# BaeHann/feature_level_style_transfer_for_TSC

Measured on AMD Instinct MI355X. Metric: train-step samples/sec (univariate TS, len=512, batch=256) at 1/2/4/8 MI355X, higher is better.
Workload: dtype bf16x3

## Files before the change

feature_level_style_transfer_for_tsc_amd/_lib.py:

```python
from __future__ import annotations

import ctypes
import os
from ctypes import POINTER, Structure, c_char_p, c_float, c_int, c_int32, c_int64, c_void_p
from typing import Optional

import torch

ABI_VERSION = 14
_LIB_NAME = "libfst_hip.so"
_HERE = os.path.dirname(os.path.abspath(__file__))
LIB_PATH = os.environ.get("FST_HIP_LIB", os.path.join(_HERE, _LIB_NAME))


class FstLibraryError(RuntimeError):
    pass


class WSrc(Structure):
    _fields_ = [("w", c_void_p), ("off0", c_int64), ("sm", c_int64), ("sc", c_int64), ("st", c_int64)]


_P = c_void_p
_I32P = c_void_p
_SIGNATURES = {
    "fst_version": (c_int, []),
    "fst_last_error": (c_char_p, []),
    "fst_pack_weights": (c_int, [_I32P, _I32P, c_int, POINTER(WSrc), POINTER(WSrc), c_int, c_int, c_int, c_int, _P, c_void_p]),
    "fst_pack_weights_bf16x3": (c_int, [_I32P, _I32P, c_int, POINTER(WSrc), POINTER(WSrc), c_int, c_int, c_int, c_int, _P, c_void_p]),
    "fst_unpack_weights": (c_int, [_I32P, _I32P, c_int, _P, c_int, _P, c_int64, c_int64, c_int64, c_int64,
                                   _P, c_int64, c_int64, c_int64, c_int64, c_int, c_void_p]),
    "fst_mask_taps": (c_int, [_P, _I32P, _I32P, c_int, c_int, c_int, c_void_p]),
    "fst_conv_gemm": (c_int, [_P, c_int64, _P, c_int64, _P, _I32P, _I32P, c_int, _P, _P, c_int64, _P, c_int64,
                              _P, c_int64, c_int, c_int, c_int, c_int, c_int, c_int, c_int, c_int, c_void_p]),
    "fst_conv_wgrad": (c_int, [_P, c_int64, _P, c_int64, _P, c_int64, _P, c_int64, c_int, _P, _I32P, _I32P, c_int,
                               c_int, c_int, c_int, c_int, c_int, c_int64, c_void_p]),
    "fst_conv_last_route": (c_int, [POINTER(c_int32)]),
    "fst_row_sum": (c_int, [_P, c_int64, c_int, c_int, c_int, _P, c_void_p]),
    "fst_bn_stats": (c_int, [_P, c_int, c_int, c_int, _P, c_int64, c_void_p]),
    "fst_bn_finalize": (c_int, [_P, c_int, _P, _P, _P, _P, c_int, c_int, c_float, c_float, _P, c_void_p]),
    "fst_bn_apply": (c_int, [_P, _P, _P, _P, _P, c_int, c_int, c_int, c_int, c_int64, c_void_p]),
    "fst_bn_bwd_reduce": (c_int, [_P, _P, _P, _P, c_int, c_int, c_int, c_int, _P, c_int64, c_void_p]),
    "fst_bn_bwd_apply": (c_int, [_P, _P, _P, _P, _P, c_int, _P, _P, _P, c_int, c_int, c_int, c_int, c_int, c_int, c_int64, c_void_p]),
    "fst_gate_fwd": (c_int, [_P, _P, c_int, c_int, c_int, c_int64, c_void_p]),
    "fst_gate_bwd": (c_int, [_P, _P, _P, c_int, c_int, c_int, c_int64, c_void_p]),
    "fst_coupling_sum_slots": (c_int64, [c_int, c_int, c_int]),
    "fst_coupling_fwd": (c_int, [_P, _P, _P, c_int, c_int, c_int, c_int64, _P, c_void_p]),
    "fst_coupling_bwd": (c_int, [_P, _P, _P, _P, _P, _P, _P, _P, c_int, c_int, c_int, c_int64, c_void_p]),
    "fst_coupling_inv_fwd": (c_int, [_P, _P, _P, c_int, c_int, c_int, c_int64, c_void_p]),
    "fst_coupling_inv_bwd": (c_int, [_P, _P, _P, _P, _P, c_int, c_int, c_int, c_int64, c_void_p]),
    "fst_rmsprop_multi": (c_int, [_P, _P, _P, _P, _P, c_int, c_float, c_float, c_void_p]),
    "fst_adam_multi": (c_int, [_P, _P, _P, _P, _P, c_int, _P, c_float, c_float, c_float, c_float, c_void_p]),
    "fst_wn_stack_fwd_ok": (c_int, [c_int, c_int, c_int, c_int]),
    "fst_wn_stack_fwd": (c_int, [_P, _P, _P, c_int64, _P, _P, _P, c_int64, _P, c_int, c_int, c_int, c_int, c_int, c_int64, c_void_p]),
    "fst_wn_stack_bwd_ok": (c_int, [c_int, c_int, c_int, c_int]),
    "fst_wn_stack_bwd": (c_int, [_P, _P, _P, _P, _P, _P, _P, _P, _P, c_int64, c_int, c_int, c_int, c_int, c_int, c_int64, c_void_p]),
    "fst_wn_wgrad_ok": (c_int, [c_int, c_int, c_int, c_int, c_int, c_int]),
    "fst_wn_wgrad_workspace_floats": (c_int64, [c_int, c_int, c_int, c_int, c_int, c_int]),
    "fst_wn_wgrad_in": (c_int, [_P, _P, _P, c_int, c_int64, _P, _P, _P, c_int64, c_int, c_int, c_int, c_int, c_int, c_int, c_int64,
                                c_void_p]),
    "fst_wn_wgrad_rs": (c_int, [_P, _P, _P, c_int, _P, _P, c_int64, c_int, c_int, c_int, c_int, c_int64, c_void_p]),
    "fst_nt_gemm_workspace_floats": (c_int64, [c_int, c_int, c_int]),
    "fst_nt_gemm": (c_int, [_P, _P, _P, _P, c_int64, c_int, c_int, c_int, _P, _P, c_int, c_float, _P, c_void_p]),
    "fst_tap_wgrad_ok": (c_int, [c_int, c_int, c_int, c_int, c_int, c_int, c_int]),
    "fst_tap_wgrad_workspace_floats": (c_int64, [c_int, c_int, c_int, c_int, c_int]),
    "fst_tap_wgrad": (c_int, [_P, _P, _P, _P, c_int64, c_int, c_int, c_int, c_int, c_int, c_int, c_int, c_int, c_int64, c_int64, c_void_p]),
# ... 93 lines not shown
```

feature_level_style_transfer_for_tsc_amd/csrc/pointwise.hip:

```cpp
#include "fst_common.h"

static thread_local char g_err[512] = "";
void fst_set_error(const char* fmt, ...) {
  va_list ap;
  va_start(ap, fmt);
  vsnprintf(g_err, sizeof(g_err), fmt, ap);
  va_end(ap);
}
extern "C" const char* fst_last_error(void) { return g_err; }

int fst_allow_full_lds(const void* fn, const char* who) {
  static const void* done[64];
  static int n_done = 0;
  for (int i = 0; i < n_done; ++i)
    if (done[i] == fn) return 0;
  hipError_t e = hipFuncSetAttribute(fn, hipFuncAttributeMaxDynamicSharedMemorySize, 160 * 1024);
  if (e != hipSuccess) {
    fst_set_error("%s: hipFuncSetAttribute: %s", who, hipGetErrorString(e));
    return (int)e;
  }
  if (n_done < 64) done[n_done++] = fn;
  return 0;
}
int fst_cu_count(void) {
// ... 184 lines not shown
    rvar[c] = (1.f - momentum) * rvar[c] + momentum * unbiased;
  } else {
    mean = rmean[c];
    var = rvar[c];
  }
  const float invstd = 1.0f / sqrtf(var + eps);
  const float scale = gamma[c] * invstd;
  stats[c] = mean;
  stats[C + c] = invstd;
  stats[2 * C + c] = scale;
  stats[3 * C + c] = beta[c] - mean * scale;
}

extern "C" int fst_bn_finalize(const float* part, int n_slots, const float* gamma, const float* beta, float* running_mean,
                               float* running_var, int train, int C, float eps, float momentum, float* stats, void* stream) {
  FST_REQUIRE(gamma && beta && running_mean && running_var && stats && C > 0, "fst_bn_finalize: bad arguments");
  FST_REQUIRE(!train || (part && n_slots > 0), "fst_bn_finalize: train mode needs the moment partials (n_slots=%d)", n_slots);
  hipLaunchKernelGGL(bn_finalize_kernel, dim3((C + 63) / 64), dim3(64), 0, (hipStream_t)stream, part, n_slots, gamma, beta,
                     running_mean, running_var, train, C, eps, momentum, stats);
  FST_LAUNCH_CHECK();
  return 0;
}

__global__ __launch_bounds__(256) void bn_apply_kernel(const float* y, const float* stats, const float* res,
                                                       const float* res_stats, float* out, int C, int L, int relu) {
  const int bc = blockIdx.x;
  const int c = bc % C;
  const float sc = stats[2 * C + c], sh = stats[3 * C + c];
  float rsc = 1.f, rsh = 0.f;
  if (res && res_stats) { rsc = res_stats[2 * C + c]; rsh = res_stats[3 * C + c]; }
  const long long base = (long long)bc * L;
  for (int t = threadIdx.x; t < L; t += 256) {
    float v = y[base + t] * sc + sh;
    if (res) v += res[base + t] * rsc + rsh;
    if (relu) v = fmaxf(v, 0.f);
    out[base + t] = v;
  }
}

__global__ __launch_bounds__(256) void bn_apply_vec_kernel(const float* y, const float* stats, const float* res,
                                                           const float* res_stats, float* out, int rows, int C, int L,
                                                           int relu, RowVec rv) {
  const int r = threadIdx.x >> rv.shift, t0 = threadIdx.x & ((1 << rv.shift) - 1), rpp = 256 >> rv.shift;
  const int bc = blockIdx.x * rpp + r;
  if (bc >= rows) return;
  const int c = bc % C;
  const float sc = stats[2 * C + c], sh = stats[3 * C + c];
  float rsc = 1.f, rsh = 0.f;
  if (res && res_stats) { rsc = res_stats[2 * C + c]; rsh = res_stats[3 * C + c]; }
  const long long base = (long long)bc * rv.L4;
  const float4* y4 = reinterpret_cast<const float4*>(y) + base;
  const float4* r4 = res ? reinterpret_cast<const float4*>(res) + base : nullptr;
  float4* o4 = reinterpret_cast<float4*>(out) + base;
  for (int t = t0; t < rv.L4; t += 1 << rv.shift) {
    float4 v = y4[t];
    v.x = v.x * sc + sh; v.y = v.y * sc + sh; v.z = v.z * sc + sh; v.w = v.w * sc + sh;
    if (r4) {
      const float4 q = r4[t];
      v.x += q.x * rsc + rsh; v.y += q.y * rsc + rsh; v.z += q.z * rsc + rsh; v.w += q.w * rsc + rsh;
    }
    if (relu) { v.x = fmaxf(v.x, 0.f); v.y = fmaxf(v.y, 0.f); v.z = fmaxf(v.z, 0.f); v.w = fmaxf(v.w, 0.f); }
    o4[t] = v;
  }
}

extern "C" int fst_bn_apply(const float* y, const float* stats, const float* res, const float* res_stats, float* out,
                            int B, int C, int L, int relu, int64_t numel, void* stream) {
  FST_REQUIRE(y && stats && out && B > 0 && C > 0 && L > 0, "fst_bn_apply: bad arguments");
  FST_REQUIRE_EXTENT("fst_bn_apply", B, C, L, numel);
  if (vec_ok(L, {y, res, out})) {
    const RowVec rv = row_vec(L);
    const int rpp = 256 >> rv.shift;
    hipLaunchKernelGGL(bn_apply_vec_kernel, dim3((B * C + rpp - 1) / rpp), dim3(256), 0, (hipStream_t)stream, y, stats, res,
                       res_stats, out, B * C, C, L, relu, rv);
  } else {
    hipLaunchKernelGGL(bn_apply_kernel, dim3(B * C), dim3(256), 0, (hipStream_t)stream, y, stats, res, res_stats, out, C, L, relu);
  }
  FST_LAUNCH_CHECK();
  return 0;
}

__global__ __launch_bounds__(256) void bn_bwd_reduce_kernel(const float* dy, const float* y, const float* out,
                                                            const float* stats, int B, int C, int L, int relu, float* red) {
  const int c = blockIdx.x;
  const float mean = stats[c], invstd = stats[C + c];
  float s1 = 0.f, s2 = 0.f;
  for (int b = blockIdx.y; b < B; b += gridDim.y) {
    const long long base = ((long long)b * C + c) * L;
    for (int t = threadIdx.x; t < L; t += 256) {
      float g = dy[base + t];
      if (relu && !(out[base + t] > 0.f)) g = 0.f;
      s1 += g;
      s2 += g * (y[base + t] - mean) * invstd;
    }
  }
  block_sum2(s1, s2);
  if (threadIdx.x == 0) {
    red[(long long)c * FST_BN_SLOTS + blockIdx.y] = s1;
    red[((long long)C + c) * FST_BN_SLOTS + blockIdx.y] = s2;
  }
}

__global__ __launch_bounds__(256) void bn_bwd_reduce_vec_kernel(const float* dy, const float* y, const float* out,
                                                                const float* stats, int B, int C, int L, int relu,
                                                                float* red, RowVec rv) {
  const int c = blockIdx.x, r = threadIdx.x >> rv.shift, t0 = threadIdx.x & ((1 << rv.shift) - 1), rpp = 256 >> rv.shift;
  const float mean = stats[c], invstd = stats[C + c];
  float s1 = 0.f, s2 = 0.f;
  for (int b = blockIdx.y + r * gridDim.y; b < B; b += rpp * gridDim.y) {
    const long long base = ((long long)b * C + c) * rv.L4;
    const float4* dy4 = reinterpret_cast<const float4*>(dy) + base;
    const float4* y4 = reinterpret_cast<const float4*>(y) + base;
    const float4* o4 = reinterpret_cast<const float4*>(out) + base;
    for (int t = t0; t < rv.L4; t += 1 << rv.shift) {
      float4 g = dy4[t];
      const float4 v = y4[t];
      if (relu) {
        const float4 o = o4[t];
        if (!(o.x > 0.f)) g.x = 0.f;
        if (!(o.y > 0.f)) g.y = 0.f;
        if (!(o.z > 0.f)) g.z = 0.f;
        if (!(o.w > 0.f)) g.w = 0.f;
      }
      s1 += (g.x + g.y) + (g.z + g.w);
      s2 += (g.x * (v.x - mean) + g.y * (v.y - mean) + g.z * (v.z - mean) + g.w * (v.w - mean)) * invstd;
    }
  }
  block_sum2(s1, s2);
  if (threadIdx.x == 0) {
    red[(long long)c * FST_BN_SLOTS + blockIdx.y] = s1;
    red[((long long)C + c) * FST_BN_SLOTS + blockIdx.y] = s2;
  }
}

extern "C" int fst_bn_bwd_reduce(const float* dy, const float* y, const float* out, const float* stats, int B, int C,
                                 int L, int relu, float* red, int64_t numel, void* stream) {
  FST_REQUIRE(dy && y && stats && red && (!relu || out) && B > 0 && C > 0 && L > 0, "fst_bn_bwd_reduce: bad arguments");
  FST_REQUIRE_EXTENT("fst_bn_bwd_reduce", B, C, L, numel);
  if (vec_ok(L, {dy, y, out}))
    hipLaunchKernelGGL(bn_bwd_reduce_vec_kernel, dim3(C, FST_BN_SLOTS), dim3(256), 0, (hipStream_t)stream, dy,
                       y, out, stats, B, C, L, relu, red, row_vec(L));
  else
    hipLaunchKernelGGL(bn_bwd_reduce_kernel, dim3(C, FST_BN_SLOTS), dim3(256), 0, (hipStream_t)stream, dy, y,
                       out, stats, B, C, L, relu, red);
  FST_LAUNCH_CHECK();
  return 0;
}

__device__ __forceinline__ void bn_red_sums(const float* red, int n_slots, int C, int c, float& r1, float& r2) {
  r1 = 0.f; r2 = 0.f;
  for (int s = 0; s < n_slots; ++s) {
    r1 += red[(long long)c * n_slots + s];
    r2 += red[((long long)C + c) * n_slots + s];
  }
}

__global__ __launch_bounds__(256) void bn_bwd_apply_kernel(const float* dy, const float* y, const float* out,
                                                           const float* stats, const float* red, int n_slots, float* red_out,
                                                           float* dx, float* row_sums, int C, int L, int relu, int train, float invN) {
  const int bc = blockIdx.x;
  const int c = bc % C;
  const float mean = stats[c], invstd = stats[C + c], scale = stats[2 * C + c];
  float r1 = 0.f, r2 = 0.f;
  if (red) bn_red_sums(red, n_slots, C, c, r1, r2);
  if (red_out && bc < C && threadIdx.x == 0) { red_out[c] = r1; red_out[C + c] = r2; }
  const float m1 = train ? r1 * invN : 0.f, m2 = train ? r2 * invN : 0.f;
  const long long base = (long long)bc * L;
  float rs = 0.f, dummy = 0.f;
  for (int t = threadIdx.x; t < L; t += 256) {
    float g = dy[base + t];
    if (relu && !(out[base + t] > 0.f)) g = 0.f;
    const float xh = (y[base + t] - mean) * invstd;
    const float d = scale * (g - m1 - xh * m2);
    dx[base + t] = d;
    rs += d;
  }
  if (row_sums) {
    block_sum2(rs, dummy);
    if (threadIdx.x == 0) row_sums[bc] = rs;
  }
}

__global__ __launch_bounds__(256) void bn_bwd_apply_vec_kernel(const float* dy, const float* y, const float* out,
                                                               const float* stats, const float* red, int n_slots,
                                                               float* red_out, float* dx, float* row_sums, int rows, int C,
                                                               int L, int relu, int train, float invN, RowVec rv) {
  __shared__ float wsum[4];
  const int r = threadIdx.x >> rv.shift, t0 = threadIdx.x & ((1 << rv.shift) - 1), rpp = 256 >> rv.shift;
  const int bc_raw = blockIdx.x * rpp + r;
  const bool live = bc_raw < rows;
  const int bc = live ? bc_raw : rows - 1;
  const int c = bc % C;
  const float mean = stats[c], invstd = stats[C + c], scale = stats[2 * C + c];
  float r1 = 0.f, r2 = 0.f;
  if (red) bn_red_sums(red, n_slots, C, c, r1, r2);
  if (red_out && live && bc < C && t0 == 0) { red_out[c] = r1; red_out[C + c] = r2; }
  const float m1 = train ? r1 * invN : 0.f, m2 = train ? r2 * invN : 0.f;
  const long long base = (long long)bc * rv.L4;
  const float4* dy4 = reinterpret_cast<const float4*>(dy) + base;
  const float4* y4 = reinterpret_cast<const float4*>(y) + base;
  const float4* o4 = reinterpret_cast<const float4*>(out) + base;
  float4* dx4 = reinterpret_cast<float4*>(dx) + base;
  float rs = 0.f;
  for (int t = t0; t < rv.L4; t += 1 << rv.shift) {
    float4 g = dy4[t];
    const float4 v = y4[t];
    if (relu) {
      const float4 o = o4[t];
      if (!(o.x > 0.f)) g.x = 0.f;
      if (!(o.y > 0.f)) g.y = 0.f;
      if (!(o.z > 0.f)) g.z = 0.f;
      if (!(o.w > 0.f)) g.w = 0.f;
    }
    float4 d;
    d.x = scale * (g.x - m1 - (v.x - mean) * invstd * m2);
    d.y = scale * (g.y - m1 - (v.y - mean) * invstd * m2);
    d.z = scale * (g.z - m1 - (v.z - mean) * invstd * m2);
    d.w = scale * (g.w - m1 - (v.w - mean) * invstd * m2);
    if (live) dx4[t] = d;
    rs += (d.x + d.y) + (d.z + d.w);
  }
  if (row_sums) {
    const int w = rv.shift < 6 ? rv.shift : 6;
    for (int o = (1 << w) >> 1; o > 0; o >>= 1) rs += __shfl_xor(rs, o, 64);
    if (rv.shift <= 6) {
      if (live && t0 == 0) row_sums[bc] = rs;
    } else {
      if ((threadIdx.x & 63) == 0) wsum[threadIdx.x >> 6] = rs;
      __syncthreads();
      if (live && t0 == 0) {
        const int w0 = threadIdx.x >> 6, nw = 1 << (rv.shift - 6);
        float tot = 0.f;
        for (int i = 0; i < nw; ++i) tot += wsum[w0 + i];
        row_sums[bc] = tot;
      }
    }
  }
}

extern "C" int fst_bn_bwd_apply(const float* dy, const float* y, const float* out, const float* stats, const float* red,
                                int n_slots, float* red_out, float* dx, float* row_sums, int B, int C, int L, int relu, int train,
                                int B_total, int64_t numel, void* stream) {
  FST_REQUIRE(dy && y && stats && dx && (!relu || out) && (!train || red), "fst_bn_bwd_apply: bad arguments");
  FST_REQUIRE(B > 0 && C > 0 && L > 0 && B_total >= B, "fst_bn_bwd_apply: B=%d C=%d L=%d B_total=%d", B, C, L, B_total);
  FST_REQUIRE(!red || n_slots > 0, "fst_bn_bwd_apply: n_slots=%d", n_slots);
  FST_REQUIRE(!red_out || red, "fst_bn_bwd_apply: red_out needs red");
  FST_REQUIRE_EXTENT("fst_bn_bwd_apply", B, C, L, numel);
  if (vec_ok(L, {dy, y, out, dx})) {
    const RowVec rv = row_vec(L);
    const int rpp = 256 >> rv.shift;
    hipLaunchKernelGGL(bn_bwd_apply_vec_kernel, dim3((B * C + rpp - 1) / rpp), dim3(256), 0, (hipStream_t)stream, dy, y, out,
                       stats, red, n_slots, red_out, dx, row_sums, B * C, C, L, relu, train, 1.0f / ((float)B_total * (float)L), rv);
  } else {
    hipLaunchKernelGGL(bn_bwd_apply_kernel, dim3(B * C), dim3(256), 0, (hipStream_t)stream, dy, y, out, stats, red, n_slots,
                       red_out, dx, row_sums, C, L, relu, train, 1.0f / ((float)B_total * (float)L));
  }
  FST_LAUNCH_CHECK();
  return 0;
}

__global__ __launch_bounds__(256) void gate_fwd_kernel(float* g, float* acts, int n, int L) {
  const int b = blockIdx.y;
  const long long total = (long long)n * L;
  float* gt = g + (long long)b * 2 * total;
  float* gs = gt + total;
  float* ab = acts + (long long)b * total;
  for (long long i = (long long)blockIdx.x * 256 + threadIdx.x; i < total; i += (long long)gridDim.x * 256) {
    const float t = tanhf(gt[i]);
    const float s = 1.0f / (1.0f + expf(-gs[i]));
    gt[i] = t;
    gs[i] = s;
    ab[i] = t * s;
  }
}

extern "C" int fst_gate_fwd(float* g_ts, float* acts, int B, int n, int L, int64_t numel_acts, void* stream) {
  FST_REQUIRE(g_ts && acts && B > 0 && n > 0 && L > 0, "fst_gate_fwd: bad arguments");
  FST_REQUIRE_EXTENT("fst_gate_fwd", B, n, L, numel_acts);
// ... 335 lines not shown
```

feature_level_style_transfer_for_tsc_amd/ops.py:

```python
from __future__ import annotations

import ctypes
import math
import os
from typing import Dict, List, Optional, Sequence, Tuple

import torch

from . import _lib
from . import dist as _dist
from ._lib import WSrc, check, ptr, stream_ptr
from .plan import Plan, Segment, build_plan, pick_mb

EPI_RELU, EPI_ACC2, EPI_ATOMIC, EPI_ACC1 = 1, 2, 4, 8
GEMM_BF16X3 = 16
WGRAD_SLABS = 32
MATH = os.environ.get("FST_MATH", "bf16x3")
LDS_BUDGET = 96 * 1024
LDS_MULTI_CHUNK = 44 * 1024
PIPE_C = 16

_PARTIAL_BACKWARD = False


# ... 683 lines not shown
    part = torch.empty(2, C, BN_SLOTS, device=y.device, dtype=torch.float32)
    check(lib.fst_bn_bwd_reduce(ptr(dy), ptr(y), ptr(out), ptr(stats), B, C, L, int(relu), ptr(part), _same_numel(dy, y, out),
                                stream_ptr()),
          "fst_bn_bwd_reduce")
    if not need_dx:
        red = part.sum(dim=2).view(2 * C)
        return None, red[C:], red[:C]
    dx = torch.empty_like(y)
    rs = torch.empty(B, C, device=y.device, dtype=torch.float32)
    if training and _dist.global_batch_active():
        red = part.sum(dim=2).view(2 * C)
        red_g = red.clone()
        B_total = _dist.sum_over_ranks_(red_g) * B
        check(lib.fst_bn_bwd_apply(ptr(dy), ptr(y), ptr(out), ptr(stats), ptr(red_g), 1, None, ptr(dx), ptr(rs), B, C, L, int(relu),
                                   int(training), B_total, _same_numel(dy, y, out, dx), stream_ptr()), "fst_bn_bwd_apply")
    else:
        red = torch.empty(2 * C, device=y.device, dtype=torch.float32)
        check(lib.fst_bn_bwd_apply(ptr(dy), ptr(y), ptr(out), ptr(stats), ptr(part), BN_SLOTS, ptr(red), ptr(dx), ptr(rs), B, C, L,
                                   int(relu), int(training), B, _same_numel(dy, y, out, dx), stream_ptr()), "fst_bn_bwd_apply")
    _ROW_SUMS.attach(dx, rs)
    return dx, red[C:], red[:C]


class BNActFn(torch.autograd.Function):

    @staticmethod
    def forward(ctx, y, gamma, beta, rmean, rvar, training: bool, relu: bool, eps: float, momentum: float):
        lib = _lib.load()
        y = y.contiguous()
        B, C, L = y.shape
        stats = _bn_stats(y, gamma, beta, rmean, rvar, training, eps, momentum)
        out = torch.empty_like(y)
        check(lib.fst_bn_apply(ptr(y), ptr(stats), None, None, ptr(out), B, C, L, int(relu), _same_numel(y, out), stream_ptr()),
              "fst_bn_apply")
        ctx.save_for_backward(y, out, stats)
        ctx.relu, ctx.training = relu, training
        return out

    @staticmethod
    def backward(ctx, dout):
        y, out, stats = ctx.saved_tensors
        dx, dg, db = _bn_backward(dout.contiguous(), y, out if ctx.relu else None, stats, ctx.relu, ctx.training,
                                  ctx.needs_input_grad[0])
        return dx, dg, db, None, None, None, None, None, None


class BNAddBNReluFn(torch.autograd.Function):

    @staticmethod
    def forward(ctx, ya, ga, ba, rma, rva, yb, gb, bb, rmb, rvb, training: bool, eps: float, momentum: float):
        lib = _lib.load()
        ya, yb = ya.contiguous(), yb.contiguous()
        B, C, L = ya.shape
        sa = _bn_stats(ya, ga, ba, rma, rva, training, eps, momentum)
        sb = _bn_stats(yb, gb, bb, rmb, rvb, training, eps, momentum)
        out = torch.empty_like(ya)
        check(lib.fst_bn_apply(ptr(ya), ptr(sa), ptr(yb), ptr(sb), ptr(out), B, C, L, 1, _same_numel(ya, yb, out), stream_ptr()),
              "fst_bn_apply")
        ctx.save_for_backward(ya, yb, out, sa, sb)
        ctx.training = training
        return out

    @staticmethod
    def backward(ctx, dout):
        ya, yb, out, sa, sb = ctx.saved_tensors
        dout = dout.contiguous()
        dxa, dga, dba = _bn_backward(dout, ya, out, sa, True, ctx.training, ctx.needs_input_grad[0])
        dxb, dgb, dbb = _bn_backward(dout, yb, out, sb, True, ctx.training, ctx.needs_input_grad[5])
        return dxa, dga, dba, None, None, dxb, dgb, dbb, None, None, None, None, None


class WNSpecs:

    def __init__(self, h: int, n: int, n_layers: int = 8, kernel: int = 3):
        self.h, self.n, self.n_layers, self.kernel = h, n, n_layers, kernel
        self.start = ConvSpec(n, h)
        self.ins = [ConvSpec(2 * n, n, kernel, 2 ** i, int((kernel * 2 ** i - 2 ** i) / 2), C1=h) for i in range(n_layers)]
        self.rs = [ConvSpec(2 * n if i < n_layers - 1 else n, n) for i in range(n_layers)]
        self.end = ConvSpec(2 * h, n)
        self.rs_T = build_plan(n, [Segment(0, n, 0, 1), Segment(1, n, 0, 1)], 1, 1, 0, chunk_c=PIPE_C)
        self.rs_T_last = build_plan(n, [Segment(0, n, 0, 1)], 1, 1, 0, chunk_c=PIPE_C)
        nl = n_layers
        self.shapes = ([(n, h, 1), (n,), (2 * n * nl, h, 1), (2 * n * nl,), (2 * h, n, 1), (2 * h,)]
                       + [(2 * n, n, kernel)] * nl + [(2 * n,)] * nl
                       + [(2 * n if i < nl - 1 else n, n, 1) for i in range(nl)] + [(2 * n if i < nl - 1 else n,) for i in range(nl)])
        self.offsets = [0]
        for sh in self.shapes:
            self.offsets.append(self.offsets[-1] + int(math.prod(sh)))
        self.flat_numel = self.offsets[-1]

    def flatten(self, weights: Sequence[Tensor]) -> Tensor:
# ... 1110 lines not shown
```

include/fst_hip.h:

```cpp
#ifndef FST_HIP_H
#define FST_HIP_H

#include <stdint.h>

#ifdef __cplusplus
extern "C" {
#endif

#define FST_ABI_VERSION 14

int fst_version(void);
const char* fst_last_error(void);

#define FST_PLAN_HEADER 16

typedef struct {
  const float* w;
  int64_t off0, sm, sc, st;
} fst_wsrc;

int fst_pack_weights(const int32_t* plan_dev, const int32_t* plan_host, int plan_len,
                     const fst_wsrc* src0_host, const fst_wsrc* src1_host,
                     int M, int g_begin, int g_end , int row_base ,
                     float* a_packed, void* stream);

int fst_pack_weights_bf16x3(const int32_t* plan_dev, const int32_t* plan_host, int plan_len,
                            const fst_wsrc* src0_host, const fst_wsrc* src1_host,
                            int M, int g_begin, int g_end, int row_base, void* a_image, void* stream);

int fst_unpack_weights(const int32_t* plan_dev, const int32_t* plan_host, int plan_len,
                       const float* a_packed, int M,
                       float* dw0, int64_t off0_0, int64_t sm0, int64_t sc0, int64_t st0,
// ... 28 lines not shown
#define FST_ROUTE_WIN_ROWS  5
#define FST_ROUTE_WGRAD     6
#define FST_ROUTE_EPI_PLAIN   0
#define FST_ROUTE_EPI_ADD     1
#define FST_ROUTE_EPI_ATOMIC  2
#define FST_ROUTE_EPI_VEC     3
#define FST_ROUTE_EPI_VEC_ADD 4
int fst_conv_last_route(int32_t out[8]);

int fst_row_sum(const float* x, int64_t x_bs, int B, int C, int L, float* out, void* stream);

#define FST_BN_SLOTS 16
int fst_bn_stats(const float* y, int B, int C, int L, float* part , int64_t numel, void* stream);
int fst_bn_finalize(const float* part, int n_slots, const float* gamma, const float* beta,
                    float* running_mean, float* running_var, int train, int C, float eps, float momentum,
                    float* stats, void* stream);
int fst_bn_apply(const float* y, const float* stats, const float* res, const float* res_stats,
                 float* out, int B, int C, int L, int relu, int64_t numel, void* stream);
int fst_bn_bwd_reduce(const float* dy, const float* y, const float* out, const float* stats,
                      int B, int C, int L, int relu, float* red , int64_t numel, void* stream);
int fst_bn_bwd_apply(const float* dy, const float* y, const float* out, const float* stats, const float* red, int n_slots,
                     float* red_out, float* dx, float* row_sums, int B, int C, int L, int relu, int train, int B_total,
                     int64_t numel, void* stream);

int fst_gate_fwd(float* g_ts, float* acts, int B, int n, int L, int64_t numel_acts, void* stream);
int fst_gate_bwd(const float* ts, const float* dacts, float* dg, int B, int n, int L, int64_t numel_acts, void* stream);
int64_t fst_coupling_sum_slots(int B, int h, int L);
int fst_coupling_fwd(const float* u, const float* o, float* xn, int B, int h, int L, int64_t numel, float* sums, void* stream);
int fst_coupling_bwd(const float* u, const float* o, const float* dxn, const float* dlogs, const float* g_ls, const float* g_sq,
                     float* du, float* d_o, int B, int h, int L, int64_t numel, void* stream);
int fst_coupling_inv_fwd(const float* x, const float* o, float* xn, int B, int h, int L, int64_t numel, void* stream);
int fst_coupling_inv_bwd(const float* xn, const float* o, const float* dxn,
                         float* dx, float* d_o, int B, int h, int L, int64_t numel, void* stream);

int fst_wn_fold_fwd(const int64_t* table_dev, int n_rows, float* flat, float* norms , void* stream);
int fst_wn_fold_bwd(const int64_t* table_dev, int n_rows, const float* d_flat, const float* norms, float* dpar, void* stream);

int fst_logdet_inv(const float* W, int n, float* out , float* inv_t , void* stream);

int64_t fst_wn_image_bytes(int n, int h);
int fst_wn_pack(const float* in_w, const float* cond_w, const float* in_b, const float* cond_b,
                const float* rs_w, const float* rs_b, int n, int h, int ntaps , int last, void* image, int64_t image_bytes, void* stream);
int fst_wn_layer_fwd(const float* a, int64_t a_bs, const float* u0, int64_t u0_bs, const void* image, int64_t image_bytes,
                     float* ts, float* acts, float* a_next, float* out, int first, int last,
                     int B, int L, int n, int h, int dil, int64_t numel_a, void* stream);

// ... 119 lines not shown
```

Baseline: 3562.

## Recompute ReLU mask in BN backward and fuse residual-join BN backward branches

BN+ReLU autograd functions no longer save the forward output. The backward kernels instead recompute the ReLU mask from y, scale and shift, with contraction disabled so the recomputed value matches the forward exactly. For the residual join (two BNs summed then ReLU), the two separate reduce and apply passes are replaced by joint kernels. These read dy once and produce both branches' partial sums, dx and row sums. The aim is to save activation memory and cut backward memory traffic and kernel launches, at the cost of a little extra arithmetic and more complex kernels.

```diff
diff --git a/feature_level_style_transfer_for_tsc_amd/_lib.py b/feature_level_style_transfer_for_tsc_amd/_lib.py
--- a/feature_level_style_transfer_for_tsc_amd/_lib.py
+++ b/feature_level_style_transfer_for_tsc_amd/_lib.py
@@ -7,7 +7,7 @@
 
 import torch
 
-ABI_VERSION = 14
+ABI_VERSION = 15
 _LIB_NAME = "libfst_hip.so"
 _HERE = os.path.dirname(os.path.abspath(__file__))
 LIB_PATH = os.environ.get("FST_HIP_LIB", os.path.join(_HERE, _LIB_NAME))
@@ -42,6 +42,9 @@
     "fst_bn_apply": (c_int, [_P, _P, _P, _P, _P, c_int, c_int, c_int, c_int, c_int64, c_void_p]),
     "fst_bn_bwd_reduce": (c_int, [_P, _P, _P, _P, c_int, c_int, c_int, c_int, _P, c_int64, c_void_p]),
     "fst_bn_bwd_apply": (c_int, [_P, _P, _P, _P, _P, c_int, _P, _P, _P, c_int, c_int, c_int, c_int, c_int, c_int, c_int64, c_void_p]),
+    "fst_bn_bwd_reduce_join": (c_int, [_P, _P, _P, _P, _P, c_int, c_int, c_int, _P, _P, c_int64, c_void_p]),
+    "fst_bn_bwd_apply_join": (c_int, [_P, _P, _P, _P, _P, _P, _P, c_int, _P, _P, _P, _P, _P, _P, c_int, c_int, c_int, c_int, c_int,
+                                      c_int64, c_void_p]),
     "fst_gate_fwd": (c_int, [_P, _P, c_int, c_int, c_int, c_int64, c_void_p]),
     "fst_gate_bwd": (c_int, [_P, _P, _P, c_int, c_int, c_int, c_int64, c_void_p]),
     "fst_coupling_sum_slots": (c_int64, [c_int, c_int, c_int]),
diff --git a/feature_level_style_transfer_for_tsc_amd/csrc/pointwise.hip b/feature_level_style_transfer_for_tsc_amd/csrc/pointwise.hip
--- a/feature_level_style_transfer_for_tsc_amd/csrc/pointwise.hip
+++ b/feature_level_style_transfer_for_tsc_amd/csrc/pointwise.hip
@@ -230,6 +230,14 @@
   return 0;
 }
 
+__device__ __forceinline__ float bn_pre(float y, float sc, float sh) { return __builtin_fmaf(y, sc, sh); }
+__device__ __forceinline__ float bn_pre_join(float ya, float sca, float sha, float yb, float scb, float shb) {
+#pragma clang fp contract(off)
+  float v = bn_pre(ya, sca, sha);
+  v += bn_pre(yb, scb, shb);
+  return v;
+}
+
 __global__ __launch_bounds__(256) void bn_apply_kernel(const float* y, const float* stats, const float* res,
                                                        const float* res_stats, float* out, int C, int L, int relu) {
   const int bc = blockIdx.x;
@@ -239,8 +247,7 @@
   if (res && res_stats) { rsc = res_stats[2 * C + c]; rsh = res_stats[3 * C + c]; }
   const long long base = (long long)bc * L;
   for (int t = threadIdx.x; t < L; t += 256) {
-    float v = y[base + t] * sc + sh;
-    if (res) v += res[base + t] * rsc + rsh;
+    float v = res ? bn_pre_join(y[base + t], sc, sh, res[base + t], rsc, rsh) : bn_pre(y[base + t], sc, sh);
     if (relu) v = fmaxf(v, 0.f);
     out[base + t] = v;
   }
@@ -262,10 +269,12 @@
   float4* o4 = reinterpret_cast<float4*>(out) + base;
   for (int t = t0; t < rv.L4; t += 1 << rv.shift) {
     float4 v = y4[t];
-    v.x = v.x * sc + sh; v.y = v.y * sc + sh; v.z = v.z * sc + sh; v.w = v.w * sc + sh;
     if (r4) {
       const float4 q = r4[t];
-      v.x += q.x * rsc + rsh; v.y += q.y * rsc + rsh; v.z += q.z * rsc + rsh; v.w += q.w * rsc + rsh;
+      v.x = bn_pre_join(v.x, sc, sh, q.x, rsc, rsh); v.y = bn_pre_join(v.y, sc, sh, q.y, rsc, rsh);
+      v.z = bn_pre_join(v.z, sc, sh, q.z, rsc, rsh); v.w = bn_pre_join(v.w, sc, sh, q.w, rsc, rsh);
+    } else {
+      v.x = bn_pre(v.x, sc, sh); v.y = bn_pre(v.y, sc, sh); v.z = bn_pre(v.z, sc, sh); v.w = bn_pre(v.w, sc, sh);
     }
     if (relu) { v.x = fmaxf(v.x, 0.f); v.y = fmaxf(v.y, 0.f); v.z = fmaxf(v.z, 0.f); v.w = fmaxf(v.w, 0.f); }
     o4[t] = v;
@@ -288,18 +297,55 @@
   return 0;
 }
 
+__device__ __forceinline__ float bn_masked(float g, float o) { return o > 0.f ? g : 0.f; }
+__device__ __forceinline__ float4 bn_masked4(float4 g, float4 o) {
+  g.x = bn_masked(g.x, o.x); g.y = bn_masked(g.y, o.y); g.z = bn_masked(g.z, o.z); g.w = bn_masked(g.w, o.w);
+  return g;
+}
+__device__ __forceinline__ float4 bn_pre4(float4 y, float sc, float sh) {
+  return make_float4(bn_pre(y.x, sc, sh), bn_pre(y.y, sc, sh), bn_pre(y.z, sc, sh), bn_pre(y.w, sc, sh));
+}
+__device__ __forceinline__ float4 bn_pre_join4(float4 ya, float sca, float sha, float4 yb, float scb, float shb) {
+  return make_float4(bn_pre_join(ya.x, sca, sha, yb.x, scb, shb), bn_pre_join(ya.y, sca, sha, yb.y, scb, shb),
+                     bn_pre_join(ya.z, sca, sha, yb.z, scb, shb), bn_pre_join(ya.w, sca, sha, yb.w, scb, shb));
+}
+__device__ __forceinline__ float bn_gx(float g, float y, float mean, float invstd) {
+#pragma clang fp contract(off)
+  return g * (y - mean) * invstd;
+}
+__device__ __forceinline__ float bn_g4(float4 g) {
+#pragma clang fp contract(off)
+  return (g.x + g.y) + (g.z + g.w);
+}
+__device__ __forceinline__ float bn_gx4(float4 g, float4 v, float mean, float invstd) {
+#pragma clang fp contract(off)
+  return (g.x * (v.x - mean) + g.y * (v.y - mean) + g.z * (v.z - mean) + g.w * (v.w - mean)) * invstd;
+}
+__device__ __forceinline__ float bn_dx_unscaled(float g, float y, float mean, float invstd, float m1, float m2) {
+#pragma clang fp contract(off)
+  const float xh = (y - mean) * invstd;
+  return __builtin_fmaf(-xh, m2, g - m1);
+}
+__device__ __forceinline__ float4 bn_dx4(float4 g, float4 v, float mean, float invstd, float scale, float m1, float m2) {
+#pragma clang fp contract(off)
+  return make_float4(scale * bn_dx_unscaled(g.x, v.x, mean, invstd, m1, m2), scale * bn_dx_unscaled(g.y, v.y, mean, invstd, m1, m2),
+                     scale * bn_dx_unscaled(g.z, v.z, mean, invstd, m1, m2), scale * bn_dx_unscaled(g.w, v.w, mean, invstd, m1, m2));
+}
+
 __global__ __launch_bounds__(256) void bn_bwd_reduce_kernel(const float* dy, const float* y, const float* out,
                                                             const float* stats, int B, int C, int L, int relu, float* red) {
+#pragma clang fp contract(off)
   const int c = blockIdx.x;
-  const float mean = stats[c], invstd = stats[C + c];
+  const float mean = stats[c], invstd = stats[C + c], sc = stats[2 * C + c], sh = stats[3 * C + c];
   float s1 = 0.f, s2 = 0.f;
   for (int b = blockIdx.y; b < B; b += gridDim.y) {
     const long long base = ((long long)b * C + c) * L;
     for (int t = threadIdx.x; t < L; t += 256) {
       float g = dy[base + t];
-      if (relu && !(out[base + t] > 0.f)) g = 0.f;
+      const float v = y[base + t];
+      if (relu) g = bn_masked(g, out ? out[base + t] : bn_pre(v, sc, sh));
       s1 += g;
-      s2 += g * (y[base + t] - mean) * invstd;
+      s2 += bn_gx(g, v, mean, invstd);
     }
   }
   block_sum2(s1, s2);
@@ -312,8 +358,9 @@
 __global__ __launch_bounds__(256) void bn_bwd_reduce_vec_kernel(const float* dy, const float* y, const float* out,
                                                                 const float* stats, int B, int C, int L, int relu,
                                                                 float* red, RowVec rv) {
+#pragma clang fp contract(off)
   const int c = blockIdx.x, r = threadIdx.x >> rv.shift, t0 = threadIdx.x & ((1 << rv.shift) - 1), rpp = 256 >> rv.shift;
-  const float mean = stats[c], invstd = stats[C + c];
+  const float mean = stats[c], invstd = stats[C + c], sc = stats[2 * C + c], sh = stats[3 * C + c];
   float s1 = 0.f, s2 = 0.f;
   for (int b = blockIdx.y + r * gridDim.y; b < B; b += rpp * gridDim.y) {
     const long long base = ((long long)b * C + c) * rv.L4;
@@ -323,15 +370,9 @@
     for (int t = t0; t < rv.L4; t += 1 << rv.shift) {
       float4 g = dy4[t];
       const float4 v = y4[t];
-      if (relu) {
-        const float4 o = o4[t];
-        if (!(o.x > 0.f)) g.x = 0.f;
-        if (!(o.y > 0.f)) g.y = 0.f;
-        if (!(o.z > 0.f)) g.z = 0.f;
-        if (!(o.w > 0.f)) g.w = 0.f;
-      }
-      s1 += (g.x + g.y) + (g.z + g.w);
-      s2 += (g.x * (v.x - mean) + g.y * (v.y - mean) + g.z * (v.z - mean) + g.w * (v.w - mean)) * invstd;
+      if (relu) g = bn_masked4(g, out ? o4[t] : bn_pre4(v, sc, sh));
+      s1 += bn_g4(g);
+      s2 += bn_gx4(g, v, mean, invstd);
     }
   }
   block_sum2(s1, s2);
@@ -343,8 +384,9 @@
 
 extern "C" int fst_bn_bwd_reduce(const float* dy, const float* y, const float* out, const float* stats, int B, int C,
                                  int L, int relu, float* red, int64_t numel, void* stream) {
-  FST_REQUIRE(dy && y && stats && red && (!relu || out) && B > 0 && C > 0 && L > 0, "fst_bn_bwd_reduce: bad arguments");
+  FST_REQUIRE(dy && y && stats && red && B > 0 && C > 0 && L > 0, "fst_bn_bwd_reduce: bad arguments");
   FST_REQUIRE_EXTENT("fst_bn_bwd_reduce", B, C, L, numel);
+  if (!relu) out = nullptr;
   if (vec_ok(L, {dy, y, out}))
     hipLaunchKernelGGL(bn_bwd_reduce_vec_kernel, dim3(C, FST_BN_SLOTS), dim3(256), 0, (hipStream_t)stream, dy,
                        y, out, stats, B, C, L, relu, red, row_vec(L));
@@ -355,6 +397,81 @@
   return 0;
 }
 
+__global__ __launch_bounds__(256) void bn_bwd_reduce_join_kernel(const float* dy, const float* ya, const float* yb,
+                                                                 const float* sa, const float* sb, int B, int C, int L,
+                                                                 float* reda, float* redb) {
+#pragma clang fp contract(off)
+  const int c = blockIdx.x;
+  const float meana = sa[c], invstda = sa[C + c], sca = sa[2 * C + c], sha = sa[3 * C + c];
+  const float meanb = sb[c], invstdb = sb[C + c], scb = sb[2 * C + c], shb = sb[3 * C + c];
+  float s1 = 0.f, s2a = 0.f, s2b = 0.f, unused = 0.f;
+  for (int b = blockIdx.y; b < B; b += gridDim.y) {
+    const long long base = ((long long)b * C + c) * L;
+    for (int t = threadIdx.x; t < L; t += 256) {
+      const float va = ya[base + t], vb = yb[base + t];
+      const float g = bn_masked(dy[base + t], bn_pre_join(va, sca, sha, vb, scb, shb));
+      s1 += g;
+      s2a += bn_gx(g, va, meana, invstda);
+      s2b += bn_gx(g, vb, meanb, invstdb);
+    }
+  }
+  block_sum2(s1, s2a);
+  block_sum2(s2b, unused);
+  if (threadIdx.x == 0) {
+    reda[(long long)c * FST_BN_SLOTS + blockIdx.y] = s1;
+    reda[((long long)C + c) * FST_BN_SLOTS + blockIdx.y] = s2a;
+    redb[(long long)c * FST_BN_SLOTS + blockIdx.y] = s1;
+    redb[((long long)C + c) * FST_BN_SLOTS + blockIdx.y] = s2b;
+  }
+}
+
+__global__ __launch_bounds__(256) void bn_bwd_reduce_join_vec_kernel(const float* dy, const float* ya, const float* yb,
+                                                                     const float* sa, const float* sb, int B, int C, int L,
+                                                                     float* reda, float* redb, RowVec rv) {
+#pragma clang fp contract(off)
+  const int c = blockIdx.x, r = threadIdx.x >> rv.shift, t0 = threadIdx.x & ((1 << rv.shift) - 1), rpp = 256 >> rv.shift;
+  const float meana = sa[c], invstda = sa[C + c], sca = sa[2 * C + c], sha = sa[3 * C + c];
+  const float meanb = sb[c], invstdb = sb[C + c], scb = sb[2 * C + c], shb = sb[3 * C + c];
+  float s1 = 0.f, s2a = 0.f, s2b = 0.f, unused = 0.f;
+  for (int b = blockIdx.y + r * gridDim.y; b < B; b += rpp * gridDim.y) {
+    const long long base = ((long long)b * C + c) * rv.L4;
+    const float4* dy4 = reinterpret_cast<const float4*>(dy) + base;
+    const float4* ya4 = reinterpret_cast<const float4*>(ya) + base;
+    const float4* yb4 = reinterpret_cast<const float4*>(yb) + base;
+    for (int t = t0; t < rv.L4; t += 1 << rv.shift) {
+      const float4 va = ya4[t], vb = yb4[t];
+      const float4 g = bn_masked4(dy4[t], bn_pre_join4(va, sca, sha, vb, scb, shb));
+      s1 += bn_g4(g);
+      s2a += bn_gx4(g, va, meana, invstda);
+      s2b += bn_gx4(g, vb, meanb, invstdb);
+    }
+  }
+  block_sum2(s1, s2a);
+  block_sum2(s2b, unused);
+  if (threadIdx.x == 0) {
+    reda[(long long)c * FST_BN_SLOTS + blockIdx.y] = s1;
+    reda[((long long)C + c) * FST_BN_SLOTS + blockIdx.y] = s2a;
+    redb[(long long)c * FST_BN_SLOTS + blockIdx.y] = s1;
+    redb[((long long)C + c) * FST_BN_SLOTS + blockIdx.y] = s2b;
+  }
+}
+
+extern "C" int fst_bn_bwd_reduce_join(const float* dy, const float* ya, const float* yb, const float* stats_a,
+                                      const float* stats_b, int B, int C, int L, float* red_a, float* red_b, int64_t numel,
+                                      void* stream) {
+  FST_REQUIRE(dy && ya && yb && stats_a && stats_b && red_a && red_b && red_a != red_b && B > 0 && C > 0 && L > 0,
+              "fst_bn_bwd_reduce_join: bad arguments");
+  FST_REQUIRE_EXTENT("fst_bn_bwd_reduce_join", B, C, L, numel);
+  if (vec_ok(L, {dy, ya, yb}))
+    hipLaunchKernelGGL(bn_bwd_reduce_join_vec_kernel, dim3(C, FST_BN_SLOTS), dim3(256), 0, (hipStream_t)stream, dy, ya, yb,
+                       stats_a, stats_b, B, C, L, red_a, red_b, row_vec(L));
+  else
+    hipLaunchKernelGGL(bn_bwd_reduce_join_kernel, dim3(C, FST_BN_SLOTS), dim3(256), 0, (hipStream_t)stream, dy, ya, yb,
+                       stats_a, stats_b, B, C, L, red_a, red_b);
+  FST_LAUNCH_CHECK();
+  return 0;
+}
+
 __device__ __forceinline__ void bn_red_sums(const float* red, int n_slots, int C, int c, float& r1, float& r2) {
   r1 = 0.f; r2 = 0.f;
   for (int s = 0; s < n_slots; ++s) {
@@ -363,12 +480,30 @@
   }
 }
 
+__device__ __forceinline__ void bn_row_sum_store(float rs, float* row_sums, int bc, bool live, int t0, RowVec rv, float* wsum) {
+  const int w = rv.shift < 6 ? rv.shift : 6;
+  for (int o = (1 << w) >> 1; o > 0; o >>= 1) rs += __shfl_xor(rs, o, 64);
+  if (rv.shift <= 6) {
+    if (live && t0 == 0) row_sums[bc] = rs;
+  } else {
+    if ((threadIdx.x & 63) == 0) wsum[threadIdx.x >> 6] = rs;
+    __syncthreads();
+    if (live && t0 == 0) {
+      const int w0 = threadIdx.x >> 6, nw = 1 << (rv.shift - 6);
+      float tot = 0.f;
+      for (int i = 0; i < nw; ++i) tot += wsum[w0 + i];
+      row_sums[bc] = tot;
+    }
+  }
+}
+
 __global__ __launch_bounds__(256) void bn_bwd_apply_kernel(const float* dy, const float* y, const float* out,
                                                            const float* stats, const float* red, int n_slots, float* red_out,
                                                            float* dx, float* row_sums, int C, int L, int relu, int train, float invN) {
+#pragma clang fp contract(off)
   const int bc = blockIdx.x;
   const int c = bc % C;
-  const float mean = stats[c], invstd = stats[C + c], scale = stats[2 * C + c];
+  const float mean = stats[c], invstd = stats[C + c], scale = stats[2 * C + c], sh = stats[3 * C + c];
   float r1 = 0.f, r2 = 0.f;
   if (red) bn_red_sums(red, n_slots, C, c, r1, r2);
   if (red_out && bc < C && threadIdx.x == 0) { red_out[c] = r1; red_out[C + c] = r2; }
@@ -377,11 +512,11 @@
   float rs = 0.f, dummy = 0.f;
   for (int t = threadIdx.x; t < L; t += 256) {
     float g = dy[base + t];
-    if (relu && !(out[base + t] > 0.f)) g = 0.f;
-    const float xh = (y[base + t] - mean) * invstd;
-    const float d = scale * (g - m1 - xh * m2);
-    dx[base + t] = d;
-    rs += d;
+    const float v = y[base + t];
+    if (relu) g = bn_masked(g, out ? out[base + t] : bn_pre(v, scale, sh));
+    const float u = bn_dx_unscaled(g, v, mean, invstd, m1, m2);
+    dx[base + t] = scale * u;
+    rs = __builtin_fmaf(scale, u, rs);
   }
   if (row_sums) {
     block_sum2(rs, dummy);
@@ -393,13 +528,14 @@
                                                                const float* stats, const float* red, int n_slots,
                                                                float* red_out, float* dx, float* row_sums, int rows, int C,
                                                                int L, int relu, int train, float invN, RowVec rv) {
+#pragma clang fp contract(off)
   __shared__ float wsum[4];
   const int r = threadIdx.x >> rv.shift, t0 = threadIdx.x & ((1 << rv.shift) - 1), rpp = 256 >> rv.shift;
   const int bc_raw = blockIdx.x * rpp + r;
   const bool live = bc_raw < rows;
   const int bc = live ? bc_raw : rows - 1;
   const int c = bc % C;
-  const float mean = stats[c], invstd = stats[C + c], scale = stats[2 * C + c];
+  const float mean = stats[c], invstd = stats[C + c], scale = stats[2 * C + c], sh = stats[3 * C + c];
   float r1 = 0.f, r2 = 0.f;
   if (red) bn_red_sums(red, n_slots, C, c, r1, r2);
   if (red_out && live && bc < C && t0 == 0) { red_out[c] = r1; red_out[C + c] = r2; }
@@ -413,47 +549,23 @@
   for (int t = t0; t < rv.L4; t += 1 << rv.shift) {
     float4 g = dy4[t];
     const float4 v = y4[t];
-    if (relu) {
-      const float4 o = o4[t];
-      if (!(o.x > 0.f)) g.x = 0.f;
-      if (!(o.y > 0.f)) g.y = 0.f;
-      if (!(o.z > 0.f)) g.z = 0.f;
-      if (!(o.w > 0.f)) g.w = 0.f;
-    }
-    float4 d;
-    d.x = scale * (g.x - m1 - (v.x - mean) * invstd * m2);
-    d.y = scale * (g.y - m1 - (v.y - mean) * invstd * m2);
-    d.z = scale * (g.z - m1 - (v.z - mean) * invstd * m2);
-    d.w = scale * (g.w - m1 - (v.w - mean) * invstd * m2);
+    if (relu) g = bn_masked4(g, out ? o4[t] : bn_pre4(v, scale, sh));
+    const float4 d = bn_dx4(g, v, mean, invstd, scale, m1, m2);
     if (live) dx4[t] = d;
-    rs += (d.x + d.y) + (d.z + d.w);
-  }
-  if (row_sums) {
-    const int w = rv.shift < 6 ? rv.shift : 6;
-    for (int o = (1 << w) >> 1; o > 0; o >>= 1) rs += __shfl_xor(rs, o, 64);
-    if (rv.shift <= 6) {
-      if (live && t0 == 0) row_sums[bc] = rs;
-    } else {
-      if ((threadIdx.x & 63) == 0) wsum[threadIdx.x >> 6] = rs;
-      __syncthreads();
-      if (live && t0 == 0) {
-        const int w0 = threadIdx.x >> 6, nw = 1 << (rv.shift - 6);
-        float tot = 0.f;
-        for (int i = 0; i < nw; ++i) tot += wsum[w0 + i];
-        row_sums[bc] = tot;
-      }
-    }
-  }
+    rs += bn_g4(d);
+  }
+  if (row_sums) bn_row_sum_store(rs, row_sums, bc, live, t0, rv, wsum);
 }
 
 extern "C" int fst_bn_bwd_apply(const float* dy, const float* y, const float* out, const float* stats, const float* red,
                                 int n_slots, float* red_out, float* dx, float* row_sums, int B, int C, int L, int relu, int train,
                                 int B_total, int64_t numel, void* stream) {
-  FST_REQUIRE(dy && y && stats && dx && (!relu || out) && (!train || red), "fst_bn_bwd_apply: bad arguments");
+  FST_REQUIRE(dy && y && stats && dx && (!train || red), "fst_bn_bwd_apply: bad arguments");
   FST_REQUIRE(B > 0 && C > 0 && L > 0 && B_total >= B, "fst_bn_bwd_apply: B=%d C=%d L=%d B_total=%d", B, C, L, B_total);
   FST_REQUIRE(!red || n_slots > 0, "fst_bn_bwd_apply: n_slots=%d", n_slots);
   FST_REQUIRE(!red_out || red, "fst_bn_bwd_apply: red_out needs red");
   FST_REQUIRE_EXTENT("fst_bn_bwd_apply", B, C, L, numel);
+  if (!relu) out = nullptr;
   if (vec_ok(L, {dy, y, out, dx})) {
     const RowVec rv = row_vec(L);
     const int rpp = 256 >> rv.shift;
@@ -462,6 +574,129 @@
   } else {
     hipLaunchKernelGGL(bn_bwd_apply_kernel, dim3(B * C), dim3(256), 0, (hipStream_t)stream, dy, y, out, stats, red, n_slots,
                        red_out, dx, row_sums, C, L, relu, train, 1.0f / ((float)B_total * (float)L));
+  }
+  FST_LAUNCH_CHECK();
+  return 0;
+}
+
+struct BnJoinBranch {
+  const float* y;
+  const float* stats;
+  const float* red;
+  float* red_out;
+  float* dx;
+  float* row_sums;
+};
+
+__global__ __launch_bounds__(256) void bn_bwd_apply_join_kernel(const float* dy, BnJoinBranch a, BnJoinBranch b, int n_slots,
+                                                                int C, int L, int train, float invN) {
+#pragma clang fp contract(off)
+  const int bc = blockIdx.x;
+  const int c = bc % C;
+  const float meana = a.stats[c], invstda = a.stats[C + c], sca = a.stats[2 * C + c], sha = a.stats[3 * C + c];
+  const float meanb = b.stats[c], invstdb = b.stats[C + c], scb = b.stats[2 * C + c], shb = b.stats[3 * C + c];
+  float ra1 = 0.f, ra2 = 0.f, rb1 = 0.f, rb2 = 0.f;
+  if (a.red) bn_red_sums(a.red, n_slots, C, c, ra1, ra2);
+  if (b.red) bn_red_sums(b.red, n_slots, C, c, rb1, rb2);
+  if (bc < C && threadIdx.x == 0) {
+    if (a.red_out) { a.red_out[c] = ra1; a.red_out[C + c] = ra2; }
+    if (b.red_out) { b.red_out[c] = rb1; b.red_out[C + c] = rb2; }
+  }
+  if (!a.dx && !b.dx) return;
+  const float ma1 = train ? ra1 * invN : 0.f, ma2 = train ? ra2 * invN : 0.f;
+  const float mb1 = train ? rb1 * invN : 0.f, mb2 = train ? rb2 * invN : 0.f;
+  const long long base = (long long)bc * L;
+  float rsa = 0.f, rsb = 0.f;
+  for (int t = threadIdx.x; t < L; t += 256) {
+    const float va = a.y[base + t], vb = b.y[base + t];
+    const float g = bn_masked(dy[base + t], bn_pre_join(va, sca, sha, vb, scb, shb));
+    if (a.dx) {
+      const float u = bn_dx_unscaled(g, va, meana, invstda, ma1, ma2);
+      a.dx[base + t] = sca * u;
+      rsa = __builtin_fmaf(sca, u, rsa);
+    }
+    if (b.dx) {
+      const float u = bn_dx_unscaled(g, vb, meanb, invstdb, mb1, mb2);
+      b.dx[base + t] = scb * u;
+      rsb = __builtin_fmaf(scb, u, rsb);
+    }
+  }
+  if (a.row_sums || b.row_sums) {
+    block_sum2(rsa, rsb);
+    if (threadIdx.x == 0) {
+      if (a.row_sums) a.row_sums[bc] = rsa;
+      if (b.row_sums) b.row_sums[bc] = rsb;
+    }
+  }
+}
+
+__global__ __launch_bounds__(256) void bn_bwd_apply_join_vec_kernel(const float* dy, BnJoinBranch a, BnJoinBranch b, int n_slots,
+                                                                    int rows, int C, int L, int train, float invN, RowVec rv) {
+#pragma clang fp contract(off)
+  __shared__ float wsum[2][4];
+  const int r = threadIdx.x >> rv.shift, t0 = threadIdx.x & ((1 << rv.shift) - 1), rpp = 256 >> rv.shift;
+  const int bc_raw = blockIdx.x * rpp + r;
+  const bool live = bc_raw < rows;
+  const int bc = live ? bc_raw : rows - 1;
+  const int c = bc % C;
+  const float meana = a.stats[c], invstda = a.stats[C + c], sca = a.stats[2 * C + c], sha = a.stats[3 * C + c];
+  const float meanb = b.stats[c], invstdb = b.stats[C + c], scb = b.stats[2 * C + c], shb = b.stats[3 * C + c];
+  float ra1 = 0.f, ra2 = 0.f, rb1 = 0.f, rb2 = 0.f;
+  if (a.red) bn_red_sums(a.red, n_slots, C, c, ra1, ra2);
+  if (b.red) bn_red_sums(b.red, n_slots, C, c, rb1, rb2);
+  if (live && bc < C && t0 == 0) {
+    if (a.red_out) { a.red_out[c] = ra1; a.red_out[C + c] = ra2; }
+    if (b.red_out) { b.red_out[c] = rb1; b.red_out[C + c] = rb2; }
+  }
+  if (!a.dx && !b.dx) return;
+  const float ma1 = train ? ra1 * invN : 0.f, ma2 = train ? ra2 * invN : 0.f;
+  const float mb1 = train ? rb1 * invN : 0.f, mb2 = train ? rb2 * invN : 0.f;
+  const long long base = (long long)bc * rv.L4;
+  const float4* dy4 = reinterpret_cast<const float4*>(dy) + base;
+  const float4* ya4 = reinterpret_cast<const float4*>(a.y) + base;
+  const float4* yb4 = reinterpret_cast<const float4*>(b.y) + base;
+  float4* dxa4 = reinterpret_cast<float4*>(a.dx) + base;
+  float4* dxb4 = reinterpret_cast<float4*>(b.dx) + base;
+  float rsa = 0.f, rsb = 0.f;
+  for (int t = t0; t < rv.L4; t += 1 << rv.shift) {
+    const float4 va = ya4[t], vb = yb4[t];
+    const float4 g = bn_masked4(dy4[t], bn_pre_join4(va, sca, sha, vb, scb, shb));
+    if (a.dx) {
+      const float4 d = bn_dx4(g, va, meana, invstda, sca, ma1, ma2);
+      if (live) dxa4[t] = d;
+      rsa += bn_g4(d);
+    }
+    if (b.dx) {
+      const float4 d = bn_dx4(g, vb, meanb, invstdb, scb, mb1, mb2);
+      if (live) dxb4[t] = d;
+      rsb += bn_g4(d);
+    }
+  }
+  if (a.row_sums) bn_row_sum_store(rsa, a.row_sums, bc, live, t0, rv, wsum[0]);
+  if (b.row_sums) bn_row_sum_store(rsb, b.row_sums, bc, live, t0, rv, wsum[1]);
+}
+
+extern "C" int fst_bn_bwd_apply_join(const float* dy, const float* ya, const float* yb, const float* stats_a,
+                                     const float* stats_b, const float* red_a, const float* red_b, int n_slots,
+                                     float* red_out_a, float* red_out_b, float* dxa, float* dxb, float* row_sums_a,
+                                     float* row_sums_b, int B, int C, int L, int train, int B_total, int64_t numel, void* stream) {
+  FST_REQUIRE(dy && ya && yb && stats_a && stats_b && (dxa || dxb || red_out_a || red_out_b), "fst_bn_bwd_apply_join: bad arguments");
+  FST_REQUIRE(!train || (red_a && red_b), "fst_bn_bwd_apply_join: train mode needs both branches' partial sums");
+  FST_REQUIRE((dxa || !row_sums_a) && (dxb || !row_sums_b), "fst_bn_bwd_apply_join: row sums of a branch without dx");
+  FST_REQUIRE(!dxa || dxa != dxb, "fst_bn_bwd_apply_join: the two dx are the same buffer");
+  FST_REQUIRE(B > 0 && C > 0 && L > 0 && B_total >= B, "fst_bn_bwd_apply_join: B=%d C=%d L=%d B_total=%d", B, C, L, B_total);
+  FST_REQUIRE((!red_a && !red_b) || n_slots > 0, "fst_bn_bwd_apply_join: n_slots=%d", n_slots);
+  FST_REQUIRE((!red_out_a || red_a) && (!red_out_b || red_b), "fst_bn_bwd_apply_join: red_out needs red");
+  FST_REQUIRE_EXTENT("fst_bn_bwd_apply_join", B, C, L, numel);
+  const BnJoinBranch a = {ya, stats_a, red_a, red_out_a, dxa, row_sums_a}, b = {yb, stats_b, red_b, red_out_b, dxb, row_sums_b};
+  const float invN = 1.0f / ((float)B_total * (float)L);
+  if (vec_ok(L, {dy, ya, yb, dxa, dxb})) {
+    const RowVec rv = row_vec(L);
+    const int rpp = 256 >> rv.shift;
+    hipLaunchKernelGGL(bn_bwd_apply_join_vec_kernel, dim3((B * C + rpp - 1) / rpp), dim3(256), 0, (hipStream_t)stream, dy, a, b,
+                       n_slots, B * C, C, L, train, invN, rv);
+  } else {
+    hipLaunchKernelGGL(bn_bwd_apply_join_kernel, dim3(B * C), dim3(256), 0, (hipStream_t)stream, dy, a, b, n_slots, C, L, train, invN);
   }
   FST_LAUNCH_CHECK();
   return 0;
diff --git a/feature_level_style_transfer_for_tsc_amd/ops.py b/feature_level_style_transfer_for_tsc_amd/ops.py
--- a/feature_level_style_transfer_for_tsc_amd/ops.py
+++ b/feature_level_style_transfer_for_tsc_amd/ops.py
@@ -729,6 +729,44 @@
     return dx, red[C:], red[:C]
 
 
+def _bn_backward_join(dy: Tensor, ya: Tensor, yb: Tensor, sa: Tensor, sb: Tensor, training: bool, need_dxa: bool,
+                      need_dxb: bool):
+    lib = _lib.load()
+    B, C, L = ya.shape
+    dev = ya.device
+    parts = torch.empty(2, 2, C, BN_SLOTS, device=dev, dtype=torch.float32)
+    check(lib.fst_bn_bwd_reduce_join(ptr(dy), ptr(ya), ptr(yb), ptr(sa), ptr(sb), B, C, L, ptr(parts[0]), ptr(parts[1]),
+                                     _same_numel(dy, ya, yb), stream_ptr()), "fst_bn_bwd_reduce_join")
+    need = (need_dxa, need_dxb)
+    dx = [torch.empty_like(y) if n else None for y, n in zip((ya, yb), need)]
+    rs = [torch.empty(B, C, device=dev, dtype=torch.float32) if n else None for n in need]
+    red = [None, None]
+    if any(need):
+        if training and _dist.global_batch_active():
+            local = parts.sum(dim=3).view(2, 2 * C)
+            red_g = local.clone()
+            B_total = _dist.sum_over_ranks_(red_g) * B
+            check(lib.fst_bn_bwd_apply_join(ptr(dy), ptr(ya), ptr(yb), ptr(sa), ptr(sb), ptr(red_g[0]), ptr(red_g[1]), 1, None, None,
+                                            ptr(dx[0]), ptr(dx[1]), ptr(rs[0]), ptr(rs[1]), B, C, L, int(training), B_total,
+                                            _same_numel(dy, ya, yb, *dx), stream_ptr()), "fst_bn_bwd_apply_join")
+            red = [local[i] if need[i] else None for i in range(2)]
+        else:
+            sums = torch.empty(2, 2 * C, device=dev, dtype=torch.float32)
+            check(lib.fst_bn_bwd_apply_join(ptr(dy), ptr(ya), ptr(yb), ptr(sa), ptr(sb), ptr(parts[0]), ptr(parts[1]), BN_SLOTS,
+                                            ptr(sums[0]) if need[0] else None, ptr(sums[1]) if need[1] else None,
+                                            ptr(dx[0]), ptr(dx[1]), ptr(rs[0]), ptr(rs[1]), B, C, L, int(training), B,
+                                            _same_numel(dy, ya, yb, *dx), stream_ptr()), "fst_bn_bwd_apply_join")
+            red = [sums[i] if need[i] else None for i in range(2)]
+    res = []
+    for i in range(2):
+        if need[i]:
+            _ROW_SUMS.attach(dx[i], rs[i])
+        else:
+            red[i] = parts[i].sum(dim=2).view(2 * C)
+        res.append((dx[i], red[i][C:], red[i][:C]))
+    return res
+
+
 class BNActFn(torch.autograd.Function):
 
     @staticmethod
@@ -740,15 +778,14 @@
         out = torch.empty_like(y)
         check(lib.fst_bn_apply(ptr(y), ptr(stats), None, None, ptr(out), B, C, L, int(relu), _same_numel(y, out), stream_ptr()),
               "fst_bn_apply")
-        ctx.save_for_backward(y, out, stats)
+        ctx.save_for_backward(y, stats)
         ctx.relu, ctx.training = relu, training
         return out
 
     @staticmethod
     def backward(ctx, dout):
-        y, out, stats = ctx.saved_tensors
-        dx, dg, db = _bn_backward(dout.contiguous(), y, out if ctx.relu else None, stats, ctx.relu, ctx.training,
-                                  ctx.needs_input_grad[0])
+        y, stats = ctx.saved_tensors
+        dx, dg, db = _bn_backward(dout.contiguous(), y, None, stats, ctx.relu, ctx.training, ctx.needs_input_grad[0])
         return dx, dg, db, None, None, None, None, None, None
 
 
@@ -764,16 +801,15 @@
         out = torch.empty_like(ya)
         check(lib.fst_bn_apply(ptr(ya), ptr(sa), ptr(yb), ptr(sb), ptr(out), B, C, L, 1, _same_numel(ya, yb, out), stream_ptr()),
               "fst_bn_apply")
-        ctx.save_for_backward(ya, yb, out, sa, sb)
+        ctx.save_for_backward(ya, yb, sa, sb)
         ctx.training = training
         return out
 
     @staticmethod
     def backward(ctx, dout):
-        ya, yb, out, sa, sb = ctx.saved_tensors
-        dout = dout.contiguous()
-        dxa, dga, dba = _bn_backward(dout, ya, out, sa, True, ctx.training, ctx.needs_input_grad[0])
-        dxb, dgb, dbb = _bn_backward(dout, yb, out, sb, True, ctx.training, ctx.needs_input_grad[5])
+        ya, yb, sa, sb = ctx.saved_tensors
+        (dxa, dga, dba), (dxb, dgb, dbb) = _bn_backward_join(dout.contiguous(), ya, yb, sa, sb, ctx.training,
+                                                             ctx.needs_input_grad[0], ctx.needs_input_grad[5])
         return dxa, dga, dba, None, None, dxb, dgb, dbb, None, None, None, None, None
 
 
diff --git a/include/fst_hip.h b/include/fst_hip.h
--- a/include/fst_hip.h
+++ b/include/fst_hip.h
@@ -7,7 +7,7 @@
 extern "C" {
 #endif
 
-#define FST_ABI_VERSION 14
+#define FST_ABI_VERSION 15
 
 int fst_version(void);
 const char* fst_last_error(void);
@@ -82,6 +82,12 @@
 int fst_bn_bwd_apply(const float* dy, const float* y, const float* out, const float* stats, const float* red, int n_slots,
                      float* red_out, float* dx, float* row_sums, int B, int C, int L, int relu, int train, int B_total,
                      int64_t numel, void* stream);
+int fst_bn_bwd_reduce_join(const float* dy, const float* ya, const float* yb, const float* stats_a, const float* stats_b,
+                           int B, int C, int L, float* red_a, float* red_b, int64_t numel, void* stream);
+int fst_bn_bwd_apply_join(const float* dy, const float* ya, const float* yb, const float* stats_a, const float* stats_b,
+                          const float* red_a, const float* red_b, int n_slots, float* red_out_a, float* red_out_b,
+                          float* dxa, float* dxb, float* row_sums_a, float* row_sums_b, int B, int C, int L, int train,
+                          int B_total, int64_t numel, void* stream);
 
 int fst_gate_fwd(float* g_ts, float* acts, int B, int n, int L, int64_t numel_acts, void* stream);
 int fst_gate_bwd(const float* ts, const float* dacts, float* dg, int B, int n, int L, int64_t numel_acts, void* stream);
```

Result: faster. 3599, median of 6 (+1.1%).
